# CWBudde/go-pocket-tts

Hardware: AMD Instinct MI355X
Metric: synthesized audio sec/sec (xRT) (higher is better)
Workload: dtype bf16; 1 GPU; b64_10s_bf16: 64 utterances/GPU x 125 frames (10.0 s each), 25-token prompt + 125-frame voice state, greedy (temperature 0), hipGraph-captured AR step, Mimi decode to 24 kHz PCM written to host; batch_per_gpu=64, frames=125, weights=BF16, kv=bf16, checkpoint=synthetic, shapes of tts_b6369a24 (seed 1234)

## Files before the change

### go-pocket-tts_amd/csrc/capi_hooks.cpp

```cpp
#include "capi_internal.h"
#include "../../include/ptts_debug.h"
#include "scan_block.h"
#include "true_peak.h"

using namespace ptts;
using namespace ptts::capi;

extern "C" {

int ptts_decode_stages(ptts_model* h, const float* latents, int32_t n_utt, int32_t frames, float* pcm, float* mimi_latent, float* transformer_out) {
    return decode_stages(h, latents, n_utt, frames, pcm, mimi_latent, transformer_out);
}

int ptts_debug_encode_stages(ptts_model* h, const float* pcm, int64_t n_samples, float* const* stages, int64_t* shapes) {
    if (stages || !shapes) {
        float* lat = stages ? stages[kEncStages - 1] : nullptr;
        std::vector<float> own;
        if (stages && !lat && h && h->m) {
            own.resize((size_t)std::max<int64_t>(ptts_mimi_encode_frames(n_samples), 1) * h->m->d.mimi_dim);
            lat = own.data();
        }
        const int rc = encode_stages(h, &pcm, &n_samples, 1, &lat, stages ? stages : nullptr);
        if (rc != PTTS_OK || !shapes) return rc;
    }
// ... 259 lines not shown
        PTTS_HIP(hipEventRecord(e1, nullptr));
        PTTS_HIP(hipEventSynchronize(e1));
        float ms = 0;
        PTTS_HIP(hipEventElapsedTime(&ms, e0, e1));
        *avg_us = ms * 1e3f / (float)iters;
        (void)hipEventDestroy(e0); (void)hipEventDestroy(e1);
        *maxdiff = -1.0f;
        if (nc <= ((size_t)200 << 20)) {
            run(variant >= 40 ? 3 : (variant >= 3 ? 2 : 3), dC2.as<float>());
            PTTS_HIP(hipDeviceSynchronize());
            std::vector<float> c1(nc), c2(nc);
            down(c1.data(), dC.p, nc * 4); down(c2.data(), dC2.p, nc * 4);
            float md = 0;
            size_t nbad = 0;
            for (size_t i = 0; i < nc; i++) {
                float d = std::fabs(c1[i] - c2[i]);
                if (!(d <= md)) md = d;
                if (d != 0 && nbad++ < 12) fprintf(stderr, "ptts_debug_gemm: variant %d vs reference at plane %zu row %zu column %zu: %.9g vs %.9g\n", variant, i / nc1, (i % nc1) / N, i % N, c1[i], c2[i]);
            }
            if (nbad) fprintf(stderr, "ptts_debug_gemm: %zu of %zu values differ from the reference kernel's\n", nbad, nc);
            for (int rep = 0; rep < 3; rep++) {
                run(variant, dC2.as<float>());
                PTTS_HIP(hipDeviceSynchronize());
                down(c2.data(), dC2.p, nc * 4);
                if (memcmp(c1.data(), c2.data(), nc * 4) != 0) {
                    size_t bad = 0, first = nc;
                    for (size_t i = 0; i < nc; i++) if (memcmp(&c1[i], &c2[i], 4) != 0) { if (first == nc) first = i; bad++; }
                    fprintf(stderr, "ptts_debug_gemm: variant %d differs from itself between runs: %zu of %zu values, first at row %zu column %zu\n", variant, bad, nc, first / N, first % N);
                    md = 1e30f;
                }
            }
            *maxdiff = md;
        }
    });
}

int ptts_debug_tall_linear(int32_t M, int32_t N, int32_t K, int32_t epi, int32_t splitk, const float* x, const float* planes, int32_t psplit, const float* pbias,
                           const float* ln_w, const float* ln_b, float eps, const float* W, const float* bias, const float* R, int32_t out_planes, float* out,
                           float* x_out) {
    return guard([&] {
        require_device();
        if (!x || !W || !out || M <= 0 || N <= 0 || K <= 0 || K % 128) throw Error(PTTS_EINVAL, "ptts_debug_tall_linear: bad arguments");
        const size_t mk = (size_t)M * K, mn = (size_t)M * N;
        const int S = std::max(1, (int)splitk);
        auto bf16 = [](float v) { uint32_t u; memcpy(&u, &v, 4); return (uint16_t)((u + 0x7fffu + ((u >> 16) & 1u)) >> 16); };
        auto f32 = [](uint16_t h) { uint32_t u = (uint32_t)h << 16; float v; memcpy(&v, &u, 4); return v; };
        const size_t nt = ((size_t)N + 15) / 16, nss = (size_t)K / 128;
        std::vector<uint16_t> wt(nt * nss * 4 * 64 * 8);
        for (size_t t = 0; t < nt; t++)
            for (size_t ss = 0; ss < nss; ss++)
                for (int sidx = 0; sidx < 4; sidx++)
                    for (int lane = 0; lane < 64; lane++)
                        for (int j = 0; j < 8; j++) {
                            const size_t n = t * 16 + (size_t)(lane & 15), k = ss * 128 + (size_t)(lane >> 4) * 32 + (size_t)sidx * 8 + j;
                            wt[((((t * nss + ss) * 4 + sidx) * 64 + lane) * 8 + j)] = n < (size_t)N ? bf16(W[n * K + k]) : 0;
                        }
        Tmp dW(wt.size() * 2), dAh(mk * 2), dAl(mk * 2), dOut((size_t)S * mn * 4), dCh(mn * 2), dCl(mn * 2);
        up(dW.p, wt.data(), wt.size() * 2);
        Tmp dB((size_t)N * 4), dR(mn * 4), dX(mk * 4), dXo(mk * 4), dP(std::max<size_t>(1, (size_t)std::max(0, (int)psplit)) * mk * 4), dPb((size_t)K * 4), dLw((size_t)K * 4), dLb((size_t)K * 4);
        if (bias) up(dB.p, bias, (size_t)N * 4);
        if (R) up(dR.p, R, mn * 4);
        if (ln_w) {
            up(dX.p, x, mk * 4); up(dLw.p, ln_w, (size_t)K * 4); up(dLb.p, ln_b, (size_t)K * 4);
            PrepArgs pa;
            pa.x = dX.as<float>(); pa.ldx = K; pa.ln_w = dLw.as<float>(); pa.ln_b = dLb.as<float>(); pa.eps = eps;
            if (planes && psplit > 0) {
// ... 160 lines not shown
```

### go-pocket-tts_amd/csrc/gemm5.hip

```cpp
#include <cstdlib>
#include <type_traits>

#include "kernels.h"
#include "device_util.h"

namespace ptts {

namespace {

typedef __bf16 bf16x8 __attribute__((ext_vector_type(8)));
typedef __bf16 bf16x2 __attribute__((ext_vector_type(2)));
typedef float f32x2 __attribute__((ext_vector_type(2)));
typedef float f32x4 __attribute__((ext_vector_type(4)));
typedef unsigned u32x4 __attribute__((ext_vector_type(4)));

union Frag5 {
    bf16x8 v;
    uint4 q;
};

__device__ __forceinline__ void split5(float a, float b, unsigned& hi, unsigned& lo) {
    f32x2 f = {a, b};
    bf16x2 h = __builtin_convertvector(f, bf16x2);
    f32x2 r = f - __builtin_convertvector(h, f32x2);
    bf16x2 l = __builtin_convertvector(r, bf16x2);
    hi = *reinterpret_cast<unsigned*>(&h);
    lo = *reinterpret_cast<unsigned*>(&l);
}

__device__ __forceinline__ int fw5(int col) { return ((col >> 3) & 1) * 3; }

template <int V> using ic = std::integral_constant<int, V>;

}

thread_local int g_gemm5_cfg = 0;

template <int BN, int NW, bool ELU_A, int ABL>
__global__ __launch_bounds__(NW * 64) __attribute__((amdgpu_waves_per_eu(2, 2))) void k_gemm5(GemmArgs a) {
    constexpr int BM = NW * 32, CH = 64, SPC = CH / 32, NTH = NW * 64, NT = BN / 16;
    constexpr int HALF = BN * 64 + 64, STAGE = SPC * HALF;
    constexpr int PPR = CH / 8, PIECES = BN * PPR, PPT = PIECES / NTH;
    static_assert(PIECES % NTH == 0, "whole 16-byte pieces per thread");
    __shared__ __attribute__((aligned(16))) char Ws[2 * STAGE];
    const int tid = threadIdx.x, lane = tid & 63, wave = tid >> 6;
    const int r16 = lane & 15, g = lane >> 4;
    const int ncol = (a.N + BN - 1) / BN, npan = (a.M + BM - 1) / BM;
    const int bid = blockIdx.x, xcd = bid & 7, jb = bid >> 3;
    const int pan = (jb / ncol) * 8 + xcd;
    if (pan >= npan) return;
    const int m0 = pan * BM + wave * 32, n0 = (jb % ncol) * BN;

    const int kz = blockIdx.y * a.kslice;
    const int KL = a.kslice ? min(a.kslice, a.K - kz) : a.K;
    const float* aptr[2];
#pragma unroll
    for (int t = 0; t < 2; t++) aptr[t] = a.A + row_off(a.amap, min(m0 + t * 16 + r16, a.M - 1)) + kz + g * 8;
    constexpr int CPP = NTH / PPR;
    const int wn = tid / PPR, wk = tid % PPR;
    const char* wsrc = (const char*)a.W + ((int64_t)(n0 + wn) * a.ldw + kz + wk * 8) * 2;
    const int64_t wstep = (int64_t)CPP * a.ldw * 2;
    const int wdst = (wk >> 2) * HALF + wn * 64 + (((wk & 3) ^ fw5(wn)) << 4);
    static_assert(CPP % 16 == 0, "");
    u32x4 wreg[PPT];
    const int wtaps = a.win_taps;
    auto koff = [&](int c) { return wtaps ? (c % wtaps) * a.win_c + (c / wtaps) * CH : c * CH; };
    auto w_load = [&](int c) {
        const int64_t ko = (int64_t)koff(c) * 2;
#pragma unroll
        for (int p = 0; p < PPT; p++) wreg[p] = *reinterpret_cast<const u32x4*>(wsrc + p * wstep + ko);
    };
    auto w_store = [&](int stage) {
#pragma unroll
        for (int p = 0; p < PPT; p++) *reinterpret_cast<u32x4*>(Ws + stage * STAGE + wdst + p * (CPP * 64)) = wreg[p];
    };

    f32x4 acc[2][NT];
#pragma unroll
    for (int t = 0; t < 2; t++)
#pragma unroll
        for (int n = 0; n < NT; n++) acc[t][n] = f32x4{0.f, 0.f, 0.f, 0.f};

    const int nchunks = KL / CH, nsteps = nchunks * SPC;
    float4 av[SPC][2][2];
    auto a_load = [&](int i, float4 (&dst)[2][2]) {
        const int ko = koff(i / SPC) + (i % SPC) * 32;
#pragma unroll
        for (int t = 0; t < 2; t++) {
            dst[t][0] = *reinterpret_cast<const float4*>(aptr[t] + ko);
            dst[t][1] = *reinterpret_cast<const float4*>(aptr[t] + ko + 4);
        }
    };
    w_load(0);
#pragma unroll
    for (int s = 0; s < SPC; s++) a_load(min(s, nsteps - 1), av[s]);
    w_store(0);
    __syncthreads();
    const int frag_off = r16 * 64 + ((g ^ fw5(r16)) << 4);
    for (int c = 0; c < nchunks; c++) {
        w_load(min(c + 1, nchunks - 1));
#pragma unroll
        for (int s = 0; s < SPC; s++) {
            const int i = c * SPC + s;
            Frag5 ah[2], al[2];
#pragma unroll
            for (int t = 0; t < 2; t++) {
                float4 x0 = av[s][t][0], x1 = av[s][t][1];
                if constexpr (ELU_A) {
                    x0.x = elu_fast(x0.x); x0.y = elu_fast(x0.y); x0.z = elu_fast(x0.z); x0.w = elu_fast(x0.w);
                    x1.x = elu_fast(x1.x); x1.y = elu_fast(x1.y); x1.z = elu_fast(x1.z); x1.w = elu_fast(x1.w);
                }
                if constexpr (ABL & 4) {
                    ah[t].q = make_uint4(__float_as_uint(x0.x), __float_as_uint(x0.y), __float_as_uint(x0.z), __float_as_uint(x0.w));
                    al[t].q = make_uint4(__float_as_uint(x1.x), __float_as_uint(x1.y), __float_as_uint(x1.z), __float_as_uint(x1.w));
                } else {
                    split5(x0.x, x0.y, ah[t].q.x, al[t].q.x);
                    split5(x0.z, x0.w, ah[t].q.y, al[t].q.y);
                    split5(x1.x, x1.y, ah[t].q.z, al[t].q.z);
                    split5(x1.z, x1.w, ah[t].q.w, al[t].q.w);
                }
            }
            if constexpr (!(ABL & 1)) a_load(min(i + SPC, nsteps - 1), av[s]);
            __builtin_amdgcn_sched_barrier(0);
// ... 10 lines not shown
                if constexpr (!(ABL & 16)) {
#pragma unroll
                    for (int t = 0; t < 2; t++) {
                        acc[t][n] = __builtin_amdgcn_mfma_f32_16x16x32_bf16(w.v, ah[t].v, acc[t][n], 0, 0, 0);
                        PTTS_LO_MFMA(acc[t][n] = __builtin_amdgcn_mfma_f32_16x16x32_bf16(w.v, al[t].v, acc[t][n], 0, 0, 0));
                    }
                } else {
                    acc[0][n][0] += __uint_as_float(w.q.x ^ ah[0].q.x ^ al[1].q.y);
                    acc[1][n][0] += __uint_as_float(w.q.y ^ ah[1].q.x ^ al[0].q.y);
                }
                if constexpr (!(ABL & 18)) {
                    __builtin_amdgcn_sched_group_barrier(0x100, 1, 0);
                    __builtin_amdgcn_sched_group_barrier(0x008, 4, 0);
                }
            }
            __builtin_amdgcn_sched_barrier(0);
        }
        w_store((c + 1) & 1);
        __syncthreads();
    }

    const float4 z4 = make_float4(0.f, 0.f, 0.f, 0.f);
    const bool has_bias = a.bias != nullptr;
    const float* bias_p = has_bias ? a.bias : reinterpret_cast<const float*>(a.W);
    auto epilogue = [&](auto epi_c, auto rope_c) {
#pragma clang fp contract(off)
        constexpr int EPI = decltype(epi_c)::value;
        constexpr bool ROPE = decltype(rope_c)::value != 0;
        constexpr bool RES = EPI >= EPI_RESADD;
        constexpr int GRP = 4;
        const bool has_scale = EPI == EPI_SCALE_RESADD && a.scale != nullptr;
        const float* scale_p = has_scale ? a.scale : reinterpret_cast<const float*>(a.W);
        const int half = a.rope_hd >> 1;
#pragma unroll
        for (int t = 0; t < 2; t++) {
            const int m = m0 + t * 16 + r16, mc = min(m, a.M - 1);
            const int64_t ro = row_off(a.cmap, mc) + blockIdx.y * a.zstride;
            int64_t tab = 0;
            if constexpr (ROPE) {
                const int pos = a.rope_row_pos ? a.rope_row_pos[mc] : a.rope_pos0 + (a.rope_rows_per_seg ? mc % a.rope_rows_per_seg : mc);
                tab = (int64_t)pos * half;
            }
            float2 cs[GRP], sn[GRP];
            if constexpr (ROPE) {
#pragma unroll
                for (int j = 0; j < GRP; j++) {
                    const int jj = ((j * 16 + 4 * g) & 63) >> 1;
                    cs[j] = *reinterpret_cast<const float2*>(a.rope_cos + tab + jj);
                    sn[j] = *reinterpret_cast<const float2*>(a.rope_sin + tab + jj);
                }
            }
#pragma unroll
            for (int nb = 0; nb < NT / GRP; nb++) {
                float4 rr[GRP], bb[GRP], sc[GRP];
#pragma unroll
                for (int j = 0; j < GRP; j++) {
                    const int cc = min(n0 + (nb * GRP + j) * 16 + 4 * g, a.N - 4);
                    bb[j] = *reinterpret_cast<const float4*>(bias_p + cc);
                    if constexpr (RES) rr[j] = *reinterpret_cast<const float4*>(a.R + ro + cc);
                    if constexpr (EPI == EPI_SCALE_RESADD) sc[j] = *reinterpret_cast<const float4*>(scale_p + cc);
                }
#pragma unroll
                for (int j = 0; j < GRP; j++) {
                    const int n = nb * GRP + j, col = n0 + n * 16 + 4 * g;
                    float4 v = make_float4(acc[t][n][0], acc[t][n][1], acc[t][n][2], acc[t][n][3]);
                    const float4 b = has_bias ? bb[j] : z4;
// ... 20 lines not shown
                    } else {
                        if (v.x == 1.2345f && m < a.M && col < a.N) *reinterpret_cast<float4*>(a.C + ro + col) = v;
                    }
                }
            }
        }
    };
    switch (a.epi) {
        case EPI_NONE:
            if (a.rope_cos && n0 < a.rope_cols) epilogue(ic<EPI_NONE>{}, ic<1>{});
            else epilogue(ic<EPI_NONE>{}, ic<0>{});
            break;
        case EPI_GELU: epilogue(ic<EPI_GELU>{}, ic<0>{}); break;
        case EPI_ELU: epilogue(ic<EPI_ELU>{}, ic<0>{}); break;
        case EPI_RESADD: epilogue(ic<EPI_RESADD>{}, ic<0>{}); break;
        case EPI_SCALE_RESADD: epilogue(ic<EPI_SCALE_RESADD>{}, ic<0>{}); break;
        case EPI_RESADD_ELU: epilogue(ic<EPI_RESADD_ELU>{}, ic<0>{}); break;
        default: break;
    }
}

bool gemm5_supported(const GemmArgs& a) {
    if (a.win_taps && (a.win_taps < 2 || a.win_c % 64 || a.K != a.win_taps * a.win_c || a.kslice)) return false;
    const bool res = a.epi >= EPI_RESADD;
    const bool epi_ok = a.epi == EPI_NONE || a.epi == EPI_GELU || a.epi == EPI_ELU || a.epi == EPI_RESADD || a.epi == EPI_SCALE_RESADD || a.epi == EPI_RESADD_ELU;
    constexpr int min_m = 1024;
    return a.w_bf16 && epi_ok && a.M >= min_m && a.K % 64 == 0 && a.K >= 64 && a.N % 128 == 0 && !a.tail &&
           (!a.kslice || (a.kslice % 64 == 0 && a.K % a.kslice == 0 && a.epi == EPI_NONE && !a.bias && !a.rope_cos && a.zstride % 4 == 0)) &&
           aligned16(a.A) && a.amap.ld % 4 == 0 && a.amap.batch_stride % 4 == 0 && a.ldw % 8 == 0 && aligned16(a.W) && (int64_t)a.N * a.ldw * 2 >= (int64_t)a.N * 4 &&
           aligned16(a.C) && a.cmap.ld % 4 == 0 && a.cmap.batch_stride % 4 == 0 && (!a.bias || aligned16(a.bias)) && (!a.scale || aligned16(a.scale)) &&
           (!res || aligned16(a.R)) && (!a.rope_cos || (a.rope_hd == 64 && a.rope_cols % 64 == 0 && a.epi == EPI_NONE));
}

template <int BN, int NW, int ABL = 0>
static void launch5_cfg(const GemmArgs& a, hipStream_t stream) {
    const int ncol = (a.N + BN - 1) / BN, npan = (a.M + NW * 32 - 1) / (NW * 32);
    dim3 grid((unsigned)(((npan + 7) / 8) * 8 * ncol), (unsigned)(a.kslice ? a.K / a.kslice : 1));
    if (a.aop == AOP_ELU) hipLaunchKernelGGL((k_gemm5<BN, NW, true, ABL>), grid, dim3(NW * 64), 0, stream, a);
    else hipLaunchKernelGGL((k_gemm5<BN, NW, false, ABL>), grid, dim3(NW * 64), 0, stream, a);
}

void launch_gemm5(const GemmArgs& a, hipStream_t stream) {
    note_launch(a.rope_cos ? "k_gemm5+rope" : a.kslice ? "k_gemm5+splitk" : "k_gemm5");
    const int cfg = g_gemm5_cfg;
    const bool wide = a.N % 256 == 0;
    switch (cfg) {
        case 1: launch5_cfg<256, 8>(a, stream); return;
        case 2: launch5_cfg<256, 4>(a, stream); return;
        case 3: launch5_cfg<128, 8>(a, stream); return;
        case 4: launch5_cfg<128, 4>(a, stream); return;
#ifdef PTTS_GEMM_PROBE
        case 11: launch5_cfg<256, 8, 1>(a, stream); return;
        case 12: launch5_cfg<256, 8, 2>(a, stream); return;
        case 14: launch5_cfg<256, 8, 4>(a, stream); return;
        case 18: launch5_cfg<256, 8, 8>(a, stream); return;
        case 26: launch5_cfg<256, 8, 16>(a, stream); return;
        case 17: launch5_cfg<256, 8, 7>(a, stream); return;
        case 25: launch5_cfg<256, 8, 15>(a, stream); return;
#endif
        default: break;
    }
    if (a.M < 16384) launch5_cfg<128, 4>(a, stream);
    else if (wide) launch5_cfg<256, 8>(a, stream);
    else launch5_cfg<128, 8>(a, stream);
}

}
// ... 1 lines not shown
```

### go-pocket-tts_amd/csrc/gemm_wres.hip

```cpp
#include <algorithm>
#include <cstdlib>

#include "kernels.h"
#include "device_util.h"

namespace ptts {

typedef __bf16 bf16x8 __attribute__((ext_vector_type(8)));
typedef __bf16 bf16x2 __attribute__((ext_vector_type(2)));
typedef float f32x2 __attribute__((ext_vector_type(2)));
typedef float f32x4 __attribute__((ext_vector_type(4)));

__device__ __forceinline__ void split2w(float a, float b, unsigned& hi, unsigned& lo) {
    f32x2 f = {a, b};
    bf16x2 h = __builtin_convertvector(f, bf16x2);
    f32x2 r = f - __builtin_convertvector(h, f32x2);
    bf16x2 l = __builtin_convertvector(r, bf16x2);
    hi = *reinterpret_cast<unsigned*>(&h);
    lo = *reinterpret_cast<unsigned*>(&l);
}

__device__ __forceinline__ int wres_fw(int col) { return ((col >> 3) & 1) * 3; }

union FragW {
    bf16x8 v;
    uint4 q;
};

constexpr int WR_RING = 4, WR_NW = 8;

template <int WR_N, int WR_K>
__global__ __launch_bounds__(WR_NW * 64) void k_gemm_wres(GemmArgs a, int ntiles, int rgl) {
    __shared__ __attribute__((aligned(16))) unsigned char Wl[WR_N * WR_K * 2];
    __shared__ __attribute__((aligned(16))) float Bl[WR_N];
    constexpr int NT = WR_N / 16;
    const int tid = threadIdx.x, lane = tid & 63, wave = __builtin_amdgcn_readfirstlane(tid >> 6);
    const int r16 = lane & 15, g = lane >> 4;
    const int xcd = blockIdx.x & 7, jb = blockIdx.x >> 3;
    const int ct = jb % ntiles, grp = xcd * rgl + jb / ntiles, ngrp = 8 * rgl;
    const int n0 = ct * WR_N;
    {
        constexpr int PPR = WR_K / 8;
        for (int pc = tid; pc < WR_N * PPR; pc += WR_NW * 64) {
            const int n = pc / PPR, kk = pc % PPR;
            uint4 u = make_uint4(0, 0, 0, 0);
            if (n0 + n < a.N && kk * 8 < a.K) u = *reinterpret_cast<const uint4*>((const char*)a.W + ((int64_t)(n0 + n) * a.ldw + kk * 8) * 2);
            *reinterpret_cast<uint4*>(Wl + (kk >> 2) * (WR_N * 64) + n * 64 + (((kk & 3) ^ wres_fw(n)) << 4)) = u;
        }
    }
    if (tid < WR_N) Bl[tid] = (a.bias && n0 + tid < a.N) ? a.bias[n0 + tid] : 0.0f;
    __syncthreads();

    const int npan = (a.M + 31) >> 5;
    const int stride = ngrp * WR_NW;
    const int p0 = grp * WR_NW + wave;
    if (p0 >= npan) return;
    const int mine = (npan - p0 + stride - 1) / stride;
    const int nsteps = a.K >> 5;
    const int total = mine * nsteps;

    float4 av[WR_RING][2][2];
    int lp = 0, li = 0;
    const float* lrow[2];
    auto l_rows = [&]() {
        const int m0 = (p0 + lp * stride) << 5;
#pragma unroll
        for (int t = 0; t < 2; t++) lrow[t] = a.A + row_off(a.amap, min(m0 + t * 16 + r16, a.M - 1)) + g * 8;
    };
    l_rows();
    auto a_load = [&](float4 (&dst)[2][2]) {
#pragma unroll
        for (int t = 0; t < 2; t++) {
            dst[t][0] = *reinterpret_cast<const float4*>(lrow[t] + li * 32);
            dst[t][1] = *reinterpret_cast<const float4*>(lrow[t] + li * 32 + 4);
        }
        if (++li == nsteps) { li = 0; lp = min(lp + 1, mine - 1); l_rows(); }
    };
#pragma unroll
    for (int r = 0; r < WR_RING; r++) a_load(av[r]);

    f32x4 acc[2][NT];
#pragma unroll
    for (int t = 0; t < 2; t++)
#pragma unroll
        for (int n = 0; n < NT; n++) acc[t][n] = f32x4{0.f, 0.f, 0.f, 0.f};

    int step = 0, pj = 0;
    for (int q0 = 0; q0 < total; q0 += WR_RING) {
#pragma unroll
        for (int r = 0; r < WR_RING; r++) {
            const int q = q0 + r;
            if (q < total) {
                FragW ah[2], al[2];
#pragma unroll
                for (int t = 0; t < 2; t++) {
                    const float4 x0 = av[r][t][0], x1 = av[r][t][1];
                    split2w(x0.x, x0.y, ah[t].q.x, al[t].q.x);
                    split2w(x0.z, x0.w, ah[t].q.y, al[t].q.y);
                    split2w(x1.x, x1.y, ah[t].q.z, al[t].q.z);
                    split2w(x1.z, x1.w, ah[t].q.w, al[t].q.w);
                }
                a_load(av[r]);
                __builtin_amdgcn_sched_barrier(0);
                const unsigned char* wb = Wl + step * (WR_N * 64) + r16 * 64 + ((g ^ wres_fw(r16)) << 4);
                FragW wh[2];
                wh[0].q = *reinterpret_cast<const uint4*>(wb);
                __builtin_amdgcn_sched_group_barrier(0x100, 1, 0);
#pragma unroll
                for (int n = 0; n < NT; n++) {
                    if (n + 1 < NT) wh[(n + 1) & 1].q = *reinterpret_cast<const uint4*>(wb + (n + 1) * 1024);
#pragma unroll
                    for (int t = 0; t < 2; t++) {
                        acc[t][n] = __builtin_amdgcn_mfma_f32_16x16x32_bf16(wh[n & 1].v, ah[t].v, acc[t][n], 0, 0, 0);
                        PTTS_LO_MFMA(acc[t][n] = __builtin_amdgcn_mfma_f32_16x16x32_bf16(wh[n & 1].v, al[t].v, acc[t][n], 0, 0, 0));
                    }
                    __builtin_amdgcn_sched_group_barrier(0x100, 1, 0);
                    __builtin_amdgcn_sched_group_barrier(0x008, 4, 0);
                }
                __builtin_amdgcn_sched_barrier(0);
                if (++step == nsteps) {
                    const int m0 = (p0 + pj * stride) << 5;
#pragma unroll
                    for (int t = 0; t < 2; t++) {
                        const int m = m0 + t * 16 + r16;
                        const int64_t ro = row_off(a.cmap, min(m, a.M - 1));
#pragma unroll
                        for (int n = 0; n < NT; n++) {
                            const int lc = n * 16 + 4 * g, col = n0 + lc;
                            float4 v = make_float4(acc[t][n][0], acc[t][n][1], acc[t][n][2], acc[t][n][3]);
                            acc[t][n] = f32x4{0.f, 0.f, 0.f, 0.f};
                            if (m >= a.M || col >= a.N) continue;
                            const float4 b = *reinterpret_cast<const float4*>(Bl + lc);
                            v.x += b.x; v.y += b.y; v.z += b.z; v.w += b.w;
                            if (a.epi == EPI_ELU) { v.x = elu_fast(v.x); v.y = elu_fast(v.y); v.z = elu_fast(v.z); v.w = elu_fast(v.w); }
                            else if (a.epi == EPI_GELU) { v.x = gelu1(v.x); v.y = gelu1(v.y); v.z = gelu1(v.z); v.w = gelu1(v.w); }
                            *reinterpret_cast<float4*>(a.C + ro + col) = v;
                        }
                    }
                    step = 0;
                    pj++;
                }
            }
        }
    }
}

static bool wres_common(const GemmArgs& a) {
    return a.w_bf16 && a.K % 32 == 0 && a.N % 4 == 0 && a.M >= 2048 && a.aop == AOP_NONE && (a.epi == EPI_NONE || a.epi == EPI_ELU || a.epi == EPI_GELU) &&
           !a.rope_cos && !a.kslice && !a.tail && aligned16(a.A) && a.amap.ld % 4 == 0 && a.amap.batch_stride % 4 == 0 && a.ldw % 8 == 0 &&
           aligned16(a.W) && aligned16(a.C) && a.cmap.ld % 4 == 0 && a.cmap.batch_stride % 4 == 0;
}
static int wres_shape(const GemmArgs& a) {
    if (!wres_common(a)) return 0;
    if (a.K <= 256 && a.K > 128 && a.N <= 256 && a.N > 128) return 1;
    if (a.K <= 512 && a.K > 256 && a.N >= 512 && (a.N + 127) / 128 <= 32 && a.M >= 16384) return 2;
    return 0;
}
bool gemm_wres_supported(const GemmArgs& a) { return wres_shape(a) != 0; }

void launch_gemm_wres(const GemmArgs& a, hipStream_t stream) {
    static const int cus = [] { int dev = 0, n = 0; (void)hipGetDevice(&dev); (void)hipDeviceGetAttribute(&n, hipDeviceAttributeMultiprocessorCount, dev); return n > 0 ? n : 256; }();
    const int per_xcd = std::max(1, cus / 8);
    note_launch(wres_shape(a) == 1 ? "k_gemm_wres<256,256>" : "k_gemm_wres<128,512>");
    if (wres_shape(a) == 1) {
        const int npan = (a.M + 31) / 32;
        const int rgl = std::max(1, std::min(per_xcd, (npan + 8 * WR_NW - 1) / (8 * WR_NW)));
        hipLaunchKernelGGL((k_gemm_wres<256, 256>), dim3((unsigned)(8 * rgl)), dim3(WR_NW * 64), 0, stream, a, 1, rgl);
    } else {
        const int ntiles = (a.N + 127) / 128;
        const int rgl = std::max(1, per_xcd / ntiles);
        hipLaunchKernelGGL((k_gemm_wres<128, 512>), dim3((unsigned)(8 * rgl * ntiles)), dim3(WR_NW * 64), 0, stream, a, ntiles, rgl);
    }
}

}
```

### go-pocket-tts_amd/runtime.py

```python
from __future__ import annotations

import ctypes as C
import os
import subprocess
import sys
from dataclasses import dataclass, field
from typing import Callable, Optional, Sequence

import numpy as np

_HERE = os.path.dirname(os.path.abspath(__file__))
LIB_PATH = os.environ.get("PTTS_LIB_PATH") or os.path.join(_HERE, "libptts_hip.so")

PTTS_OK, PTTS_EINVAL, PTTS_EIO, PTTS_EFORMAT, PTTS_ENODEVICE, PTTS_ECANCELLED, PTTS_ENOMEM = range(7)
WEIGHTS_F32, WEIGHTS_BF16, WEIGHTS_INT8 = 0, 1, 2
KV_F32, KV_BF16 = 0, 1
PCM_F32, PCM_S16, PCM_ULAW, PCM_ALAW = 0, 1, 2, 3
_PCM_DTYPES = {PCM_F32: "<f4", PCM_S16: "<i2", PCM_ULAW: "|u1", PCM_ALAW: "|u1"}

_FP = C.POINTER(C.c_float)
_IP = C.POINTER(C.c_int64)
_DP = C.POINTER(C.c_double)
_STEP_CB = C.CFUNCTYPE(None, C.c_void_p, C.c_int32, C.c_int32)
_PCM_CB = C.CFUNCTYPE(None, C.c_void_p, C.c_int64, C.c_int64, C.c_void_p)
# ... 87 lines not shown
    _fields_ = [("data", C.POINTER(C.c_float)), ("count", C.c_int64), ("rank", C.c_int32), ("reserved", C.c_int32), ("shape", C.c_int64 * 8)]


_lib = None

ABI_SYMBOLS = [
    "ptts_default_opts", "ptts_model_open", "ptts_model_open_bytes", "ptts_model_close", "ptts_model_info", "ptts_last_error",
    "ptts_plan_create", "ptts_plan_create_bytes", "ptts_plan_arena_bytes", "ptts_model_open_planned", "ptts_plan_free",
    "ptts_generate", "ptts_free_result", "ptts_text_embeddings", "ptts_batch_new", "ptts_batch_free", "ptts_batch_reset",
    "ptts_batch_set_voice_state", "ptts_batch_prompt", "ptts_batch_step", "ptts_batch_offsets", "ptts_batch_read_kv",
    "ptts_decode_latents", "ptts_noise_rows", "ptts_speaker_project", "ptts_mimi_encode", "ptts_mimi_encode_frames", "ptts_voice_encode_audio", "ptts_flow_direction", "ptts_op_linear", "ptts_op_layernorm", "ptts_op_rope",
    "ptts_op_attention_positions", "ptts_op_conv1d_leftpad", "ptts_op_convtr1d_righttrim", "ptts_version",
        "ptts_voice_create", "ptts_voice_free", "ptts_profile_enable", "ptts_profile_read", "ptts_plan_fill_host", "ptts_wav_header_streaming", "ptts_op_pcm16",
    "ptts_dispatcher_create", "ptts_dispatcher_create_custom", "ptts_dispatch_generate", "ptts_dispatcher_stats", "ptts_dispatcher_close",
    "ptts_model_share", "ptts_model_replicate", "ptts_model_set_use_graph", "ptts_model_set_max_batch", "ptts_text_estimate_max_frames", "ptts_text_frames_after_eos", "ptts_text_prepare", "ptts_text_chunks", "ptts_chunks_count",
    "ptts_chunks_get", "ptts_chunks_free",
    "ptts_tokenizer_open", "ptts_tokenizer_open_bytes", "ptts_tokenizer_free", "ptts_tokenizer_vocab_size", "ptts_tokenizer_encode",
    "ptts_tokenizer_encode_cb", "ptts_text_nfkc", "ptts_rccl_unique_id", "ptts_rccl_broadcast", "ptts_dsp_apply",
    "ptts_voice_file_open", "ptts_voice_file_open_bytes", "ptts_voice_file_close", "ptts_voice_file_kind", "ptts_voice_file_embedding",
    "ptts_voice_file_modules", "ptts_voice_file_module", "ptts_voice_file_state", "ptts_voice_open", "ptts_voice_open_bytes",
    "ptts_voice_from_embeddings", "ptts_voice_from_audio", "ptts_voice_offset", "ptts_voice_read_state", "ptts_voice_write", "ptts_voice_write_bytes",
    "ptts_voice_state_write_bytes", "ptts_voice_embedding_write", "ptts_free_bytes",
    "ptts_resample_length", "ptts_resample", "ptts_pcm_encode", "ptts_mimi_encode_rates", "ptts_voice_from_audio_rates", "ptts_wav_header",
    "ptts_dsp_rows", "ptts_loudness", "ptts_loudness_normalize", "ptts_loudness_rows", "ptts_loudness_normalize_rows",
    "ptts_eq_design", "ptts_eq_response", "ptts_eq_create", "ptts_eq_free", "ptts_eq_apply", "ptts_eq_rows",
    "ptts_dsp_ext_create", "ptts_dsp_ext_free", "ptts_true_peak", "ptts_true_peak_limit", "ptts_true_peak_rows",
    "ptts_dsp_ext_set_compressor", "ptts_compress_gain", "ptts_compress_apply", "ptts_compress_rows",
    ]
HOOK_SYMBOLS = [
    "ptts_decode_stages", "ptts_mimi_layer_piece", "ptts_debug_last_attention_kernel", "ptts_debug_launch_counts", "ptts_debug_flow_cluster_inject",
    "ptts_debug_time_skinny", "ptts_debug_skinny_stamps", "ptts_debug_gemm", "ptts_debug_step_stamps", "ptts_debug_tall_linear",
    "ptts_debug_encode_stages", "ptts_debug_resample_launches", "ptts_debug_dsp_blocked_host",
    "ptts_debug_loudness_energies", "ptts_debug_kweighting", "ptts_debug_step_linear", "ptts_debug_true_peak_taps", "ptts_debug_true_peak_oversample",
    "ptts_debug_dsp_opts_error",
]


def build(force: bool = False) -> str:
    args = ["make", "-s", "-C", _HERE, "-j8"]
    if force:
        args.append("-B")
    subprocess.check_call(args)
    return LIB_PATH


def lib():
    global _lib
    if _lib is None:
        if not os.path.exists(LIB_PATH):
            raise PttsError(PTTS_ENODEVICE, f"{LIB_PATH} is missing: run __graft_entry__.build() (no CPU fallback exists)")
        if "torch" not in sys.modules and not os.environ.get("PTTS_NO_TORCH_PRELOAD"):
            try:
                import torch
            except Exception:
                pass
        L = C.CDLL(LIB_PATH)
        L.ptts_last_error.restype = C.c_char_p
        L.ptts_version.restype = C.c_char_p
        L.ptts_plan_arena_bytes.restype = C.c_size_t
        L.ptts_plan_arena_bytes.argtypes = [C.c_void_p]
        L.ptts_plan_free.argtypes = [C.c_void_p]
        L.ptts_model_close.argtypes = [C.c_void_p]
        L.ptts_batch_free.argtypes = [C.c_void_p]
        L.ptts_model_open.argtypes = [C.c_char_p, C.POINTER(_Opts), C.POINTER(C.c_void_p)]
        L.ptts_model_open_bytes.argtypes = [C.c_void_p, C.c_size_t, C.POINTER(_Opts), C.POINTER(C.c_void_p)]
        L.ptts_plan_create.argtypes = [C.c_char_p, C.POINTER(_Opts), C.POINTER(C.c_void_p)]
        L.ptts_plan_create_bytes.argtypes = [C.c_void_p, C.c_size_t, C.POINTER(_Opts), C.POINTER(C.c_void_p)]
# ... 1535 lines not shown
```

### include/ptts_debug.h

```cpp
#ifndef PTTS_DEBUG_H
#define PTTS_DEBUG_H

#include "ptts.h"

#ifdef __cplusplus
extern "C" {
#endif

#define PTTS_MIMI_PIECE_QKV 0
#define PTTS_MIMI_PIECE_FFN 1
int  ptts_mimi_layer_piece(ptts_model* m, int32_t layer, int32_t which, const float* x, int64_t rows, int32_t pos0, int32_t rows_per_seg, float* out);

int  ptts_decode_stages(ptts_model* m, const float* latents, int32_t n_utt, int32_t frames,
                        float* pcm, float* mimi_latent, float* transformer_out);

int  ptts_debug_encode_stages(ptts_model* m, const float* pcm, int64_t n_samples, float* const* stages, int64_t* shapes);

int ptts_debug_time_skinny(int32_t M, int32_t N, int32_t K, int32_t w_bf16, int32_t splitk, int32_t fuse_ln, int32_t iters, float* avg_us);
int ptts_debug_skinny_stamps(int32_t M, int32_t N, int32_t K, int32_t w_bf16, int32_t splitk, int32_t fuse_ln, uint64_t* out ,
                             int32_t max_blocks, int32_t* n_blocks);
int ptts_debug_step_stamps(ptts_batch* b, int32_t lsd_steps, uint64_t* out , int64_t cap_blocks, int32_t* desc ,
                           int32_t cap_desc, int32_t* n_desc);
int ptts_debug_gemm(int32_t M, int32_t N, int32_t K, int32_t w_bf16, int32_t variant, int32_t epi, int32_t iters, float* avg_us,
                    float* maxdiff);

int ptts_debug_tall_linear(int32_t M, int32_t N, int32_t K, int32_t epi, int32_t splitk, const float* x, const float* planes, int32_t psplit, const float* pbias,
                           const float* ln_w, const float* ln_b, float eps, const float* W, const float* bias, const float* R, int32_t out_planes, float* out,
                           float* x_out);

typedef struct ptts_step_linear_args {
    int32_t M, N, K, lda, ldc, wfmt, epi, splitk, tail, path, ldg, ln, ldmod, psplit, r_in_c, zrows, pgate, reserved;
    float alpha, eps;
    const float *x, *W, *bias, *addvec, *R, *scale, *gate, *ln_w, *ln_b, *shift, *mscale, *planes, *pbias;
    float *C, *tail_out, *x_out, *y_out, *w_eff, *w_scale;
    int32_t* launches;
} ptts_step_linear_args;
int ptts_debug_step_linear(const ptts_step_linear_args* a);

const char* ptts_debug_last_attention_kernel(void);

int64_t ptts_debug_launch_counts(int32_t on, char* out, int64_t cap);
int64_t ptts_debug_resample_launches(int32_t reset);

int ptts_debug_dsp_blocked_host(const float* in, int64_t n, float* out);

int ptts_debug_loudness_energies(ptts_model* m, const float* const* in, const int64_t* n, int32_t rows, double* const* out);
int ptts_debug_kweighting(int32_t sample_rate, double out[10]);

int ptts_debug_flow_cluster_inject(ptts_model* m, int32_t block);


int64_t ptts_debug_dsp_opts_error(const ptts_dsp_opts* opts, char* out, int64_t cap);
int ptts_debug_true_peak_taps(float* out , int32_t* L, int32_t* K, int32_t* dlo);
int ptts_debug_true_peak_oversample(const float* samples, int64_t n, float* y );

#ifdef __cplusplus
}
// ... 3 lines not shown
```

Measured before the change: 12780 x real-time.

## Transpose GEMM epilogue tiles through LDS for row-contiguous stores

The gemm5 and weight-resident GEMM epilogues now pass each wave's MFMA accumulator fragments through a small per-wave LDS slot, so every lane writes a float4 of a row-contiguous 32-column span instead of scattered 16-column fragments. This is meant to make output and residual traffic coalesce better. The cost is extra LDS round trips and wave barriers in the epilogue, plus an extra LDS slot in the wres kernel that may reduce occupancy. Compile-time ABL flags also add an alternative A-load pattern and a store-suppression probe mode, and a debug entry point compares whole versus row-sliced GEMM launches.

New measurement: 12780 x real-time (median of 5 runs). No clear change (+0.0%).

```diff
diff --git a/go-pocket-tts_amd/csrc/capi_hooks.cpp b/go-pocket-tts_amd/csrc/capi_hooks.cpp
--- a/go-pocket-tts_amd/csrc/capi_hooks.cpp
+++ b/go-pocket-tts_amd/csrc/capi_hooks.cpp
@@ -315,6 +315,55 @@
             }
             *maxdiff = md;
         }
+    });
+}
+
+int ptts_debug_gemm_rows(int32_t M, int32_t N, int32_t K, const float* A, int64_t a_elems, const int64_t a_map[4], const float* W, const float* bias,
+                         const float* scale, const float* c_init, int64_t c_elems, const int64_t c_map[4], int32_t epi, int32_t aop, int32_t win_taps,
+                         int32_t win_c, int32_t slice, float* out_whole, float* out_sliced) {
+    return guard([&] {
+        require_device();
+        if (!A || !W || !a_map || !c_map || !c_init || !out_whole || !out_sliced || M <= 0 || N <= 0 || K <= 0 || slice <= 0 || a_elems <= 0 || c_elems <= 0)
+            throw Error(PTTS_EINVAL, "ptts_debug_gemm_rows: bad arguments");
+        auto last = [&](const int64_t* mp, int64_t width) {
+            int64_t top = 0;
+            for (int64_t r = 0; r < M; r++) top = std::max(top, mp[0] + (mp[2] ? (r / mp[2]) * mp[3] + (r % mp[2]) * mp[1] : r * mp[1]) + width);
+            return top;
+        };
+        for (int i = 0; i < 4; i++) if (a_map[i] < 0 || c_map[i] < 0) throw Error(PTTS_EINVAL, "ptts_debug_gemm_rows: negative map entry");
+        if (last(a_map, K) > a_elems || last(c_map, N) > c_elems) throw Error(PTTS_EINVAL, "ptts_debug_gemm_rows: the row map leaves its buffer");
+        const size_t nw = (size_t)N * K;
+        std::vector<uint16_t> hw16(nw);
+        for (size_t i = 0; i < nw; i++) { uint32_t u; memcpy(&u, &W[i], 4); hw16[i] = (uint16_t)((u + 0x7fffu + ((u >> 16) & 1u)) >> 16); }
+        Tmp dA((size_t)a_elems * 4), dW(nw * 2), dB((size_t)N * 4), dS((size_t)N * 4), dC((size_t)c_elems * 4);
+        up(dA.p, A, (size_t)a_elems * 4); up(dW.p, hw16.data(), nw * 2);
+        if (bias) up(dB.p, bias, (size_t)N * 4);
+        if (scale) up(dS.p, scale, (size_t)N * 4);
+        GemmArgs g;
+        g.A = dA.as<float>() + a_map[0]; g.amap = RowMap{a_map[1], a_map[2], a_map[3]};
+        g.W = dW.p; g.w_bf16 = 1; g.ldw = K; g.bias = bias ? dB.as<float>() : nullptr; g.scale = scale ? dS.as<float>() : nullptr;
+        g.C = dC.as<float>() + c_map[0]; g.cmap = RowMap{c_map[1], c_map[2], c_map[3]};
+        g.R = g.C; g.epi = epi; g.aop = aop; g.win_taps = win_taps; g.win_c = win_c;
+        g.M = M; g.N = N; g.K = K;
+        up(dC.p, c_init, (size_t)c_elems * 4);
+        launch_gemm(g, nullptr);
+        PTTS_HIP(hipDeviceSynchronize());
+        down(out_whole, dC.p, (size_t)c_elems * 4);
+        up(dC.p, c_init, (size_t)c_elems * 4);
+        const int64_t seg_rows = a_map[2] ? a_map[2] : M;
+        if (c_map[2] && c_map[2] != seg_rows) throw Error(PTTS_EINVAL, "ptts_debug_gemm_rows: the two maps' segments differ");
+        for (int64_t s0 = 0; s0 < M; s0 += seg_rows)
+            for (int64_t r0 = s0; r0 < std::min<int64_t>(M, s0 + seg_rows); r0 += slice) {
+                GemmArgs h = g;
+                h.M = (int)std::min<int64_t>(slice, std::min<int64_t>(M, s0 + seg_rows) - r0);
+                const int64_t b = r0 / seg_rows, t = r0 - b * seg_rows;
+                h.A = g.A + (a_map[2] ? b * a_map[3] : 0) + t * a_map[1]; h.amap = RowMap{a_map[1], 0, 0};
+                h.C = g.C + (c_map[2] ? b * c_map[3] : 0) + t * c_map[1]; h.cmap = RowMap{c_map[1], 0, 0};
+                h.R = h.C;
+                launch_gemm(h, nullptr);
+            }
+        PTTS_HIP(hipDeviceSynchronize());
+        down(out_sliced, dC.p, (size_t)c_elems * 4);
     });
 }
 
diff --git a/go-pocket-tts_amd/csrc/gemm5.hip b/go-pocket-tts_amd/csrc/gemm5.hip
--- a/go-pocket-tts_amd/csrc/gemm5.hip
+++ b/go-pocket-tts_amd/csrc/gemm5.hip
@@ -3,6 +3,7 @@
 
 #include "kernels.h"
 #include "device_util.h"
+#include "wave_transpose.h"
 
 namespace ptts {
 
@@ -53,9 +54,15 @@
 
     const int kz = blockIdx.y * a.kslice;
     const int KL = a.kslice ? min(a.kslice, a.K - kz) : a.K;
-    const float* aptr[2];
-#pragma unroll
-    for (int t = 0; t < 2; t++) aptr[t] = a.A + row_off(a.amap, min(m0 + t * 16 + r16, a.M - 1)) + kz + g * 8;
+    constexpr int NAP = (ABL & 32) ? 4 : 2;
+    const float* aptr[NAP];
+    if constexpr (ABL & 32) {
+#pragma unroll
+        for (int j = 0; j < 4; j++) aptr[j] = a.A + row_off(a.amap, min(m0 + j * 8 + (lane >> 3), a.M - 1)) + kz + (lane & 7) * 4;
+    } else {
+#pragma unroll
+        for (int t = 0; t < 2; t++) aptr[t] = a.A + row_off(a.amap, min(m0 + t * 16 + r16, a.M - 1)) + kz + g * 8;
+    }
     constexpr int CPP = NTH / PPR;
     const int wn = tid / PPR, wk = tid % PPR;
     const char* wsrc = (const char*)a.W + ((int64_t)(n0 + wn) * a.ldw + kz + wk * 8) * 2;
@@ -85,10 +92,15 @@
     float4 av[SPC][2][2];
     auto a_load = [&](int i, float4 (&dst)[2][2]) {
         const int ko = koff(i / SPC) + (i % SPC) * 32;
-#pragma unroll
-        for (int t = 0; t < 2; t++) {
-            dst[t][0] = *reinterpret_cast<const float4*>(aptr[t] + ko);
-            dst[t][1] = *reinterpret_cast<const float4*>(aptr[t] + ko + 4);
+        if constexpr (ABL & 32) {
+#pragma unroll
+            for (int j = 0; j < 4; j++) dst[j >> 1][j & 1] = *reinterpret_cast<const float4*>(aptr[j] + ko);
+        } else {
+#pragma unroll
+            for (int t = 0; t < 2; t++) {
+                dst[t][0] = *reinterpret_cast<const float4*>(aptr[t] + ko);
+                dst[t][1] = *reinterpret_cast<const float4*>(aptr[t] + ko + 4);
+            }
         }
     };
     w_load(0);
@@ -165,6 +177,73 @@
         const bool has_scale = EPI == EPI_SCALE_RESADD && a.scale != nullptr;
         const float* scale_p = has_scale ? a.scale : reinterpret_cast<const float*>(a.W);
         const int half = a.rope_hd >> 1;
+        if constexpr (!ROPE) {
+            unsigned char* const slot = reinterpret_cast<unsigned char*>(Ws) + wave * kWtSlotBytes;
+            static_assert(NW * kWtSlotBytes <= 2 * STAGE, "the slots fit in the weight stages");
+            const int pc = wt_piece(lane);
+#pragma unroll
+            for (int t = 0; t < 2; t++) {
+                int mr[2];
+                int64_t ro[2];
+#pragma unroll
+                for (int h = 0; h < 2; h++) {
+                    mr[h] = m0 + t * 16 + wt_row(lane, h);
+                    ro[h] = row_off(a.cmap, min(mr[h], a.M - 1)) + blockIdx.y * a.zstride;
+                }
+#pragma unroll
+                for (int nb = 0; nb < NT / 4; nb++) {
+                    float4 rr[2][2], bb[2], sc[2], cur[2][2];
+#pragma unroll
+                    for (int j = 0; j < 2; j++) {
+                        const int cc = min(n0 + (nb * 2 + j) * 32 + 4 * pc, a.N - 4);
+                        bb[j] = *reinterpret_cast<const float4*>(bias_p + cc);
+                        if constexpr (EPI == EPI_SCALE_RESADD) sc[j] = *reinterpret_cast<const float4*>(scale_p + cc);
+                        if constexpr (RES) {
+#pragma unroll
+                            for (int h = 0; h < 2; h++) rr[j][h] = *reinterpret_cast<const float4*>(a.R + ro[h] + cc);
+                        }
+                    }
+#pragma unroll
+                    for (int j = 0; j < 2; j++) {
+#pragma unroll
+                        for (int nn = 0; nn < 2; nn++) {
+                            const int n = (nb * 2 + j) * 2 + nn;
+                            wt_put(slot, lane, nn, make_float4(acc[t][n][0], acc[t][n][1], acc[t][n][2], acc[t][n][3]));
+                        }
+                        wt_sync();
+#pragma unroll
+                        for (int h = 0; h < 2; h++) cur[j][h] = wt_get(slot, lane, h);
+                        wt_sync();
+                    }
+#pragma unroll
+                    for (int j = 0; j < 2; j++) {
+                        const int col = n0 + (nb * 2 + j) * 32 + 4 * pc;
+                        const float4 b = has_bias ? bb[j] : z4;
+#pragma unroll
+                        for (int h = 0; h < 2; h++) {
+                            float4 v = cur[j][h];
+                            v.x += b.x; v.y += b.y; v.z += b.z; v.w += b.w;
+                            if constexpr (EPI == EPI_GELU) { v.x = gelu1(v.x); v.y = gelu1(v.y); v.z = gelu1(v.z); v.w = gelu1(v.w); }
+                            if constexpr (EPI == EPI_ELU) { v.x = elu_fast(v.x); v.y = elu_fast(v.y); v.z = elu_fast(v.z); v.w = elu_fast(v.w); }
+                            if constexpr (EPI == EPI_RESADD) { v.x = rr[j][h].x + v.x; v.y = rr[j][h].y + v.y; v.z = rr[j][h].z + v.z; v.w = rr[j][h].w + v.w; }
+                            if constexpr (EPI == EPI_SCALE_RESADD) {
+                                const float4 s = has_scale ? sc[j] : make_float4(1.f, 1.f, 1.f, 1.f);
+                                v.x = rr[j][h].x + s.x * v.x; v.y = rr[j][h].y + s.y * v.y; v.z = rr[j][h].z + s.z * v.z; v.w = rr[j][h].w + s.w * v.w;
+                            }
+                            if constexpr (EPI == EPI_RESADD_ELU) {
+                                v.x = elu_fast(rr[j][h].x + v.x); v.y = elu_fast(rr[j][h].y + v.y); v.z = elu_fast(rr[j][h].z + v.z); v.w = elu_fast(rr[j][h].w + v.w);
+                            }
+                            if constexpr (!(ABL & 8)) {
+                                if (mr[h] < a.M && col < a.N) *reinterpret_cast<float4*>(a.C + ro[h] + col) = v;
+                            } else {
+                                if (v.x == 1.2345f && mr[h] < a.M && col < a.N) *reinterpret_cast<float4*>(a.C + ro[h] + col) = v;
+                            }
+                        }
+                    }
+                }
+            }
+            return;
+        }
 #pragma unroll
         for (int t = 0; t < 2; t++) {
             const int m = m0 + t * 16 + r16, mc = min(m, a.M - 1);
@@ -251,7 +330,11 @@
            (!res || aligned16(a.R)) && (!a.rope_cos || (a.rope_hd == 64 && a.rope_cols % 64 == 0 && a.epi == EPI_NONE));
 }
 
-template <int BN, int NW, int ABL = 0>
+#ifndef PTTS_GEMM_ABL
+#define PTTS_GEMM_ABL 0
+#endif
+
+template <int BN, int NW, int ABL = PTTS_GEMM_ABL>
 static void launch5_cfg(const GemmArgs& a, hipStream_t stream) {
     const int ncol = (a.N + BN - 1) / BN, npan = (a.M + NW * 32 - 1) / (NW * 32);
     dim3 grid((unsigned)(((npan + 7) / 8) * 8 * ncol), (unsigned)(a.kslice ? a.K / a.kslice : 1));
diff --git a/go-pocket-tts_amd/csrc/gemm_wres.hip b/go-pocket-tts_amd/csrc/gemm_wres.hip
--- a/go-pocket-tts_amd/csrc/gemm_wres.hip
+++ b/go-pocket-tts_amd/csrc/gemm_wres.hip
@@ -3,6 +3,7 @@
 
 #include "kernels.h"
 #include "device_util.h"
+#include "wave_transpose.h"
 
 namespace ptts {
 
@@ -29,16 +30,18 @@
 
 constexpr int WR_RING = 4, WR_NW = 8;
 
-template <int WR_N, int WR_K>
+template <int WR_N, int WR_K, int ABL>
 __global__ __launch_bounds__(WR_NW * 64) void k_gemm_wres(GemmArgs a, int ntiles, int rgl) {
     __shared__ __attribute__((aligned(16))) unsigned char Wl[WR_N * WR_K * 2];
     __shared__ __attribute__((aligned(16))) float Bl[WR_N];
+    __shared__ __attribute__((aligned(16))) unsigned char Tl[WR_NW * kWtSlotBytes];
     constexpr int NT = WR_N / 16;
     const int tid = threadIdx.x, lane = tid & 63, wave = __builtin_amdgcn_readfirstlane(tid >> 6);
     const int r16 = lane & 15, g = lane >> 4;
     const int xcd = blockIdx.x & 7, jb = blockIdx.x >> 3;
     const int ct = jb % ntiles, grp = xcd * rgl + jb / ntiles, ngrp = 8 * rgl;
     const int n0 = ct * WR_N;
+    unsigned char* const slot = Tl + wave * kWtSlotBytes;
     {
         constexpr int PPR = WR_K / 8;
         for (int pc = tid; pc < WR_N * PPR; pc += WR_NW * 64) {
@@ -61,18 +64,29 @@
 
     float4 av[WR_RING][2][2];
     int lp = 0, li = 0;
-    const float* lrow[2];
+    constexpr int NLR = (ABL & 32) ? 4 : 2;
+    const float* lrow[NLR];
     auto l_rows = [&]() {
         const int m0 = (p0 + lp * stride) << 5;
-#pragma unroll
-        for (int t = 0; t < 2; t++) lrow[t] = a.A + row_off(a.amap, min(m0 + t * 16 + r16, a.M - 1)) + g * 8;
+        if constexpr (ABL & 32) {
+#pragma unroll
+            for (int j = 0; j < 4; j++) lrow[j] = a.A + row_off(a.amap, min(m0 + j * 8 + (lane >> 3), a.M - 1)) + (lane & 7) * 4;
+        } else {
+#pragma unroll
+            for (int t = 0; t < 2; t++) lrow[t] = a.A + row_off(a.amap, min(m0 + t * 16 + r16, a.M - 1)) + g * 8;
+        }
     };
     l_rows();
     auto a_load = [&](float4 (&dst)[2][2]) {
-#pragma unroll
-        for (int t = 0; t < 2; t++) {
-            dst[t][0] = *reinterpret_cast<const float4*>(lrow[t] + li * 32);
-            dst[t][1] = *reinterpret_cast<const float4*>(lrow[t] + li * 32 + 4);
+        if constexpr (ABL & 32) {
+#pragma unroll
+            for (int j = 0; j < 4; j++) dst[j >> 1][j & 1] = *reinterpret_cast<const float4*>(lrow[j] + li * 32);
+        } else {
+#pragma unroll
+            for (int t = 0; t < 2; t++) {
+                dst[t][0] = *reinterpret_cast<const float4*>(lrow[t] + li * 32);
+                dst[t][1] = *reinterpret_cast<const float4*>(lrow[t] + li * 32 + 4);
+            }
         }
         if (++li == nsteps) { li = 0; lp = min(lp + 1, mine - 1); l_rows(); }
     };
@@ -120,23 +134,48 @@
                 __builtin_amdgcn_sched_barrier(0);
                 if (++step == nsteps) {
                     const int m0 = (p0 + pj * stride) << 5;
-#pragma unroll
-                    for (int t = 0; t < 2; t++) {
-                        const int m = m0 + t * 16 + r16;
-                        const int64_t ro = row_off(a.cmap, min(m, a.M - 1));
-#pragma unroll
-                        for (int n = 0; n < NT; n++) {
-                            const int lc = n * 16 + 4 * g, col = n0 + lc;
+                    const int pc = wt_piece(lane);
+                    int mr[2][2];
+                    int64_t ro[2][2];
+#pragma unroll
+                    for (int t = 0; t < 2; t++)
+#pragma unroll
+                        for (int h = 0; h < 2; h++) {
+                            mr[t][h] = m0 + t * 16 + wt_row(lane, h);
+                            ro[t][h] = row_off(a.cmap, min(mr[t][h], a.M - 1));
+                        }
+                    float4 pend[2];
+                    auto flush = [&](int t, int np) {
+                        const int col = n0 + np * 32 + pc * 4;
+#pragma unroll
+                        for (int h = 0; h < 2; h++) {
+                            if constexpr (ABL & 8) { if (pend[h].x != 1.2345f) continue; }
+                            if (mr[t][h] < a.M && col < a.N) *reinterpret_cast<float4*>(a.C + ro[t][h] + col) = pend[h];
+                        }
+                    };
+#pragma unroll
+                    for (int p = 0; p < NT; p++) {
+                        const int t = p / (NT / 2), np = p % (NT / 2);
+#pragma unroll
+                        for (int nn = 0; nn < 2; nn++) {
+                            const int n = np * 2 + nn, lc = n * 16 + 4 * g;
                             float4 v = make_float4(acc[t][n][0], acc[t][n][1], acc[t][n][2], acc[t][n][3]);
                             acc[t][n] = f32x4{0.f, 0.f, 0.f, 0.f};
-                            if (m >= a.M || col >= a.N) continue;
                             const float4 b = *reinterpret_cast<const float4*>(Bl + lc);
                             v.x += b.x; v.y += b.y; v.z += b.z; v.w += b.w;
                             if (a.epi == EPI_ELU) { v.x = elu_fast(v.x); v.y = elu_fast(v.y); v.z = elu_fast(v.z); v.w = elu_fast(v.w); }
                             else if (a.epi == EPI_GELU) { v.x = gelu1(v.x); v.y = gelu1(v.y); v.z = gelu1(v.z); v.w = gelu1(v.w); }
-                            *reinterpret_cast<float4*>(a.C + ro + col) = v;
+                            wt_put(slot, lane, nn, v);
                         }
+                        wt_sync();
+                        float4 cur[2];
+#pragma unroll
+                        for (int h = 0; h < 2; h++) cur[h] = wt_get(slot, lane, h);
+                        wt_sync();
+                        if (p > 0) flush((p - 1) / (NT / 2), (p - 1) % (NT / 2));
+                        pend[0] = cur[0]; pend[1] = cur[1];
                     }
+                    flush(1, NT / 2 - 1);
                     step = 0;
                     pj++;
                 }
@@ -157,6 +196,10 @@
     return 0;
 }
 bool gemm_wres_supported(const GemmArgs& a) { return wres_shape(a) != 0; }
+
+#ifndef PTTS_GEMM_ABL
+#define PTTS_GEMM_ABL 0
+#endif
 
 void launch_gemm_wres(const GemmArgs& a, hipStream_t stream) {
     static const int cus = [] { int dev = 0, n = 0; (void)hipGetDevice(&dev); (void)hipDeviceGetAttribute(&n, hipDeviceAttributeMultiprocessorCount, dev); return n > 0 ? n : 256; }();
@@ -165,11 +208,11 @@
     if (wres_shape(a) == 1) {
         const int npan = (a.M + 31) / 32;
         const int rgl = std::max(1, std::min(per_xcd, (npan + 8 * WR_NW - 1) / (8 * WR_NW)));
-        hipLaunchKernelGGL((k_gemm_wres<256, 256>), dim3((unsigned)(8 * rgl)), dim3(WR_NW * 64), 0, stream, a, 1, rgl);
+        hipLaunchKernelGGL((k_gemm_wres<256, 256, PTTS_GEMM_ABL>), dim3((unsigned)(8 * rgl)), dim3(WR_NW * 64), 0, stream, a, 1, rgl);
     } else {
         const int ntiles = (a.N + 127) / 128;
         const int rgl = std::max(1, per_xcd / ntiles);
-        hipLaunchKernelGGL((k_gemm_wres<128, 512>), dim3((unsigned)(8 * rgl * ntiles)), dim3(WR_NW * 64), 0, stream, a, ntiles, rgl);
+        hipLaunchKernelGGL((k_gemm_wres<128, 512, PTTS_GEMM_ABL>), dim3((unsigned)(8 * rgl * ntiles)), dim3(WR_NW * 64), 0, stream, a, ntiles, rgl);
     }
 }
 
diff --git a/go-pocket-tts_amd/csrc/wave_transpose.h b/go-pocket-tts_amd/csrc/wave_transpose.h
--- /dev/null
+++ b/go-pocket-tts_amd/csrc/wave_transpose.h
@@ -0,0 +1,24 @@
+#pragma once
+
+#include <hip/hip_runtime.h>
+
+namespace ptts {
+
+constexpr int kWtSlotBytes = 16 * 128;
+
+__device__ __forceinline__ void wt_put(unsigned char* slot, int lane, int nn, float4 v) {
+    const int r16 = lane & 15, g = lane >> 4;
+    *reinterpret_cast<float4*>(slot + r16 * 128 + (((g + 4 * nn) ^ (r16 & 7)) << 4)) = v;
+}
+__device__ __forceinline__ int wt_row(int lane, int h) { return 8 * h + (lane >> 3); }
+__device__ __forceinline__ int wt_piece(int lane) { return (lane & 7) ^ (lane >> 3); }
+__device__ __forceinline__ float4 wt_get(const unsigned char* slot, int lane, int h) {
+    return *reinterpret_cast<const float4*>(slot + (8 * h + (lane >> 3)) * 128 + ((lane & 7) << 4));
+}
+__device__ __forceinline__ void wt_sync() {
+    __builtin_amdgcn_fence(__ATOMIC_RELEASE, "wavefront");
+    __builtin_amdgcn_wave_barrier();
+    __builtin_amdgcn_fence(__ATOMIC_ACQUIRE, "wavefront");
+}
+
+}
diff --git a/go-pocket-tts_amd/runtime.py b/go-pocket-tts_amd/runtime.py
--- a/go-pocket-tts_amd/runtime.py
+++ b/go-pocket-tts_amd/runtime.py
@@ -143,7 +143,7 @@
     "ptts_debug_time_skinny", "ptts_debug_skinny_stamps", "ptts_debug_gemm", "ptts_debug_step_stamps", "ptts_debug_tall_linear",
     "ptts_debug_encode_stages", "ptts_debug_resample_launches", "ptts_debug_dsp_blocked_host",
     "ptts_debug_loudness_energies", "ptts_debug_kweighting", "ptts_debug_step_linear", "ptts_debug_true_peak_taps", "ptts_debug_true_peak_oversample",
-    "ptts_debug_dsp_opts_error",
+    "ptts_debug_dsp_opts_error", "ptts_debug_gemm_rows",
 ]
 
 
diff --git a/include/ptts_debug.h b/include/ptts_debug.h
--- a/include/ptts_debug.h
+++ b/include/ptts_debug.h
@@ -23,6 +23,10 @@
                            int32_t cap_desc, int32_t* n_desc);
 int ptts_debug_gemm(int32_t M, int32_t N, int32_t K, int32_t w_bf16, int32_t variant, int32_t epi, int32_t iters, float* avg_us,
                     float* maxdiff);
+
+int ptts_debug_gemm_rows(int32_t M, int32_t N, int32_t K, const float* A, int64_t a_elems, const int64_t a_map[4], const float* W, const float* bias,
+                         const float* scale, const float* c_init, int64_t c_elems, const int64_t c_map[4], int32_t epi, int32_t aop, int32_t win_taps,
+                         int32_t win_c, int32_t slice, float* out_whole, float* out_sliced);
 
 int ptts_debug_tall_linear(int32_t M, int32_t N, int32_t K, int32_t epi, int32_t splitk, const float* x, const float* planes, int32_t psplit, const float* pbias,
                            const float* ln_w, const float* ln_b, float eps, const float* W, const float* bias, const float* R, int32_t out_planes, float* out,
```
